# Sliwson/cuda-slam

Measured on AMD Instinct MI355X. Metric: icp_iterations_per_s, higher is better.
Workload: dtype f32

## Files before the change

### cuda-slam_amd/csrc/context.h

```cpp
#pragma once
#include <hip/hip_runtime.h>
#include <rccl/rccl.h>
#include <sys/resource.h>

#include <cstdarg>
#include <cstdio>
#include <string>
#include <vector>

#include "../../include/mi_slam.h"
#include "cpd_kernels.h"
#include "devbuf.h"
#include "kernels.h"
#include "nn_grid.h"
#include "nn_tree.h"

namespace mislam {

void retire_buffers(struct ::mi_ctx* ctx);

#define MI_NCCL(call)                                                                                      \
    do {                                                                                                   \
        ncclResult_t r_ = (call);                                                                          \
        if (r_ != ncclSuccess) {                                                                           \
            mislam::set_error("%s failed: %s (%s:%d)", #call, ncclGetErrorString(r_), __FILE__, __LINE__); \
            return MI_ERR_RCCL;                                                                            \
        }                                                                                                  \
    } while (0)

#define MI_TRY(call)             \
    do {                         \
        int rc_ = (call);        \
        if (rc_ != MI_OK) return rc_; \
    } while (0)

struct GridBuffers {
    DevBuf<float4> pts;
    DevBuf<unsigned int> start, fill, scan;
    DevBuf<unsigned int> slot_of;
    DevBuf<unsigned int> row_occ;
    DevBuf<unsigned char> near_tmp;
};
int grid_reserve(GridBuffers& b, const float bbox[6], int m, int index_base, float points_per_cell, NnGridView* view);
int grid_build_into(GridBuffers& b, const NnGridView& view, const float* x, const float* y, const float* z, int m, hipStream_t s);

struct MortonScratch {
    DevBuf<unsigned int> codes_in, codes_out;
    DevBuf<int> order_in;
    DevBuf<float> bbox;
    DevBuf<unsigned char> sort_temp;
};
int morton_args(MortonScratch& sc, const float* x, const float* y, const float* z, int m, int* order_out, MortonArgs* out);

struct SearchFrontBuffers {
    DevBuf<float> staging;
    DevBuf<float> cx, cy, cz;
    DevBuf<float> ux, uy, uz;
    DevBuf<float> qx, qy, qz;
    DevBuf<float> range_lo_hi;
    DevBuf<int> range_bad;
    DevBuf<KnnState> state;
    DevBuf<int> order;
    MortonScratch morton;
    GridBuffers cells;
    hipEvent_t ev[2] = {nullptr, nullptr};
};

struct ProfileSpan {
    int kernel;
    hipEvent_t e0, e1;
};

struct CpdWorkspace;
struct PrepState;

}

struct mi_ctx {
    int device = 0;
    std::vector<void*> retired;
    unsigned long long entered = 0;
    hipStream_t stream = nullptr;
    int rank = 0, world = 1;
    ncclComm_t comm = nullptr;
    mi_exchange_fn exchange = nullptr;
    void* exchange_user = nullptr;
    void* exchange_host = nullptr;
    size_t exchange_cap = 0;
    bool distributed() const { return comm != nullptr || exchange != nullptr; }
    int cu_count = 256;
    struct Tuning {
        int nn_force_mode = 0;
        int nn_R = 2, nn_wgs = 0, nn_chunks = 0;
        float grid_points_per_cell = mislam::GRID_POINTS_PER_CELL;
        int cpd_mfma = 1;
        int cpd_trunc_cull = 1;
        int fgt_resume = 1;
        int grid_split_walks = -1;
        int grid_deal_rows = -1;
        int svd_ieee = 0;
        int icp_fused_solve = 1;
        int icp_ticket_solve = 1;
        int icp_pipeline = 1;
        int fgt_two_streams = 1;
        int fgt_lists_in_model = 1;
        int fgt_coop_sweep = 1;
        int fgt_shard_queries = 1;
        int fgt_model_splits = 1;
        float knn_points_per_cell = 0.f;
        float outlier_radius_cell = 1.f;
        int fgt_replay = 1;
    } tune;

    hipStream_t aux = nullptr, aux2 = nullptr;
    hipEvent_t aux_event[3] = {nullptr, nullptr, nullptr};
    hipStream_t lane_stream = nullptr;
    int lane = 0;
    hipStream_t work_stream() const { return lane_stream ? lane_stream : stream; }
    struct LaneScratch {
        mislam::DevBuf<float> staging;
        mislam::MortonScratch morton;
    } scratch[2];

    struct PinnedRing {
        static constexpr int SLOTS = 16;
        static constexpr size_t PIECE = 1u << 20;
        char* buf = nullptr;
        hipEvent_t event[SLOTS] = {nullptr};
        unsigned int busy = 0;
        unsigned int next = 0;
    } pin;
    float* h_scratch = nullptr;
    mislam::DevBuf<float> bx, by, bz;
    mislam::DevBuf<float> cx, cy, cz;
    mislam::DevBuf<float> ax, ay, az;
    mislam::DevBuf<float> tx, ty, tz;
    mislam::DevBuf<float4> tgt4;
    mislam::DevBuf<unsigned long long> keys;
    mislam::DevBuf<double> part_mom, part_err;
    struct WorkOrder {
        mislam::DevBuf<int> order, counters;
        mislam::DevBuf<int> ticket;
        mislam::DevBuf<unsigned char> far;
        mislam::DevBuf<unsigned long long> lanes;
    } sched;
    mislam::DevBuf<double> rows, rows_reduced;
    mislam::DevBuf<int> idx_tmp;
    mislam::DevBuf<unsigned char> keep_tmp;
    mislam::IcpState* d_state = nullptr;
    mislam::IcpState* h_state = nullptr;
    hipEvent_t peek_event = nullptr;

    struct TreeIndex {
        mislam::DevBuf<int> order_out;
        mislam::DevBuf<float4> pts, boxes;
        mislam::DevBuf<float4> leaf;
        mislam::DevBuf<int> idx;
        mislam::DevBuf<float> boxes6;
        mislam::NnTreeView view{};
        bool valid = false;
    } tree;
    struct GridIndex {
        mislam::GridBuffers cells;
        mislam::DevBuf<float> bbox;
        mislam::DevBuf<unsigned int> match_slot;
        mislam::NnGridView view{};
        bool valid = false;
    } grid;
    mislam::DevBuf<int> sorder;
    mislam::DevBuf<int> sinv;
    mislam::DevBuf<float> resid;

    struct BatchBuffers {
        mislam::DevBuf<float> before, after, sx, sy, sz;
        mislam::DevBuf<mislam::IcpBatchProblem> problems;
        mislam::DevBuf<mislam::IcpState> states;
        mislam::DevBuf<mislam::CpdBatchProblem> cpd_problems;
        mislam::DevBuf<mislam::CpdState> cpd_states;
        mislam::DevBuf<int> running;
    } bat;

    struct VoxelBuffers {
        mislam::DevBuf<float> staging, x, y, z, range_lo_hi, out_xyz;
        mislam::DevBuf<float4> pts;
        mislam::DevBuf<unsigned int> keys_a, keys_b, axis_keys;
        mislam::DevBuf<int> vals_a, vals_b, range_bad, block_heads, row_of, run_start, fix, out_count, out_coord, voxel_of_point;
        mislam::DevBuf<double> front, back;
        mislam::DevBuf<unsigned char> sort_temp;
        mislam::DevBuf<mislam::VoxState> state;
        double ms[MI_VOXEL_STAGES] = {0};
    } vox;

    struct KnnBuffers {
        mislam::SearchFrontBuffers front;
        mislam::DevBuf<float> out_d2;
        mislam::DevBuf<int> out_idx, out_count;
        double ms[MI_KNN_STAGES] = {0};
    } knn;
    struct NormalsBuffers {
        mislam::SearchFrontBuffers front;
        mislam::DevBuf<float> out_normals, out_curvature;
        mislam::DevBuf<int> out_count;
        double ms[MI_NORMALS_STAGES] = {0};
    } normals;
    struct OutlierBuffers {
        mislam::SearchFrontBuffers front;
        mislam::DevBuf<float> out_xyz, out_mean;
        mislam::DevBuf<int> count, tile_counts, out_index;
        mislam::DevBuf<double> score, partials;
        mislam::DevBuf<unsigned char> keep;
        mislam::DevBuf<mislam::OutlierState> ostate;
        double ms[MI_OUTLIER_STAGES] = {0};
    } outlier;

    struct PrepareBuffers {
        mislam::DevBuf<float> raw, out, partials, noise_unit, outlier_unit;
        mislam::DevBuf<int> sub, shuffle, rows;
        mislam::DevBuf<mislam::PrepState> state;
    } prep;

    struct IcpProblem {
        bool icp_loaded = false;
        int n = 0, n_pad = 0;
        int n_global = 0;
        int m_total = 0, shard_lo = 0, shard_hi = 0;
        bool source_sharded = false;
        bool fused = false;
        int enqueued_passes = 0;
        mi_icp_params icp{};
        double load_ms[MI_LOAD_STAGES] = {0};
    } prob;

    mislam::CpdWorkspace* cpd = nullptr;

    mislam::DevBuf<unsigned long long> nn_stats;
    bool nn_stats_on = false;
    int selftest_fail_loads = 0;
    struct Profiler {
// ... 162 lines not shown
```

### cuda-slam_amd/csrc/mislam_api.hip

```cpp
#include <hip/hip_runtime.h>
#include <dlfcn.h>
#include <rccl/rccl.h>

#include <algorithm>
#include <atomic>
#include <chrono>
#include <cmath>
#include <cstdio>
#include <cstdlib>
#include <cstring>
#include <mutex>
#include <vector>

#include "cloud_range.hpp"
#include "context.h"

using namespace mislam;

namespace mislam {
static thread_local char g_error[512] = "";
void set_error(const char* fmt, ...)
{
    va_list ap;
    va_start(ap, fmt);
// ... 102 lines not shown
        (void)hipMemPoolTrimTo(g_pool[dev], 0);
    }
}
void retire_buffers(mi_ctx* ctx)
{
    std::vector<void*> v;
    v.swap(ctx->retired);
    for (void* p : v) device_free(p);
}
}

double mislam::g_stall_ms = -1.0;

extern "C" const char* mi_last_error(void) { return g_error; }
extern "C" int mi_abi_version(void) { return MI_SLAM_ABI_VERSION; }

extern "C" int mi_device_count(int* count)
{
    if (!count) { set_error("mi_device_count: null argument"); return MI_ERR_INVALID_ARG; }
    int c = 0;
    hipError_t e = hipGetDeviceCount(&c);
    if (e != hipSuccess || c <= 0) {
        *count = 0;
        set_error("no usable HIP device (%s); this library has no CPU fallback", e == hipSuccess ? "count = 0" : hipGetErrorString(e));
        return MI_ERR_NO_DEVICE;
    }
    *count = c;
    return MI_OK;
}

extern "C" int mi_ctx_preload(mi_ctx* c)
{
    if (!c) { set_error("mi_ctx_preload: null context"); return MI_ERR_INVALID_ARG; }
    MI_ENTER(c);
    MI_HIP(preload_nn_kernel()); MI_HIP(preload_nn_tree()); MI_HIP(preload_nn_grid()); MI_HIP(preload_icp_kernels()); MI_HIP(preload_icp_batch()); MI_HIP(preload_cpd_kernels()); MI_HIP(preload_cpd_batch());
    MI_HIP(preload_cpd_fgt()); MI_HIP(preload_nicp_api()); MI_HIP(preload_prepare_api()); MI_HIP(preload_voxel_kernels()); MI_HIP(preload_knn_kernels()); MI_HIP(preload_normals_kernels()); MI_HIP(preload_outlier_kernels());
    return MI_OK;
}

static int ctx_create_common(int device, mi_ctx** out)
{
    if (!out) { set_error("mi_ctx_create: null out pointer"); return MI_ERR_INVALID_ARG; }
    *out = nullptr;
    int count = 0;
    MI_TRY(mi_device_count(&count));
    if (device < 0 || device >= count) { set_error("mi_ctx_create: device %d out of range [0,%d)", device, count); return MI_ERR_INVALID_ARG; }
    MI_HIP(hipSetDevice(device));
    mi_ctx* c = new mi_ctx();
    c->device = device;
    pool_context_created(device);
    const int rc = [&]() -> int {
        hipDeviceProp_t prop;
        MI_HIP(hipGetDeviceProperties(&prop, device));
        c->cu_count = prop.multiProcessorCount > 0 ? prop.multiProcessorCount : 256;
        MI_HIP(hipStreamCreateWithFlags(&c->stream, hipStreamNonBlocking));
        MI_HIP(hipStreamCreateWithFlags(&c->aux, hipStreamNonBlocking));
        MI_HIP(hipStreamCreateWithFlags(&c->aux2, hipStreamNonBlocking));
        for (hipEvent_t& e : c->aux_event) MI_HIP(hipEventCreateWithFlags(&e, hipEventDisableTiming));
        MI_HIP(hipMalloc((void**)&c->d_state, sizeof(IcpState)));
        MI_HIP(hipHostMalloc((void**)&c->h_state, sizeof(IcpState), hipHostMallocDefault));
        MI_HIP(hipEventCreateWithFlags(&c->peek_event, hipEventDisableTiming));
        memset(c->h_state, 0, sizeof(IcpState));
        auto env_i = [](const char* name, int dflt) { const char* v = getenv(name); return (v && *v) ? atoi(v) : dflt; };
        if (const char* sm = getenv("MISLAM_DEV_STALL_MS")) g_stall_ms = atof(sm);
        c->tune.nn_force_mode = env_i("MISLAM_NN_MODE", 0);
        c->tune.nn_R = env_i("MISLAM_NN_R", 2);
        c->tune.nn_wgs = env_i("MISLAM_NN_WGS", 0);
        c->tune.nn_chunks = env_i("MISLAM_NN_CHUNKS", 0);
        c->tune.cpd_mfma = env_i("MISLAM_CPD_MFMA", 1);
        c->tune.cpd_trunc_cull = env_i("MISLAM_CPD_TRUNC_CULL", 1);
        c->tune.fgt_resume = env_i("MISLAM_FGT_RESUME", 1);
        c->tune.fgt_replay = env_i("MISLAM_FGT_REPLAY", 1);
        c->tune.fgt_two_streams = env_i("MISLAM_FGT_TWO_STREAMS", 1);
        c->tune.fgt_lists_in_model = env_i("MISLAM_FGT_LISTS_IN_MODEL", 1);
        c->tune.fgt_coop_sweep = env_i("MISLAM_FGT_COOP_SWEEP", 1);
        c->tune.fgt_model_splits = env_i("MISLAM_FGT_MODEL_SPLITS", 1);
        c->tune.fgt_shard_queries = env_i("MISLAM_FGT_SHARD_QUERIES", 1);
        c->tune.grid_deal_rows = env_i("MISLAM_GRID_DEAL_ROWS", -1);
        c->tune.grid_split_walks = env_i("MISLAM_GRID_SPLIT_WALKS", -1);
        c->tune.icp_pipeline = env_i("MISLAM_ICP_PIPELINE", 1);
        c->tune.icp_fused_solve = env_i("MISLAM_ICP_FUSED_SOLVE", 1);
        c->tune.icp_ticket_solve = env_i("MISLAM_ICP_TICKET_SOLVE", 1);
        c->tune.svd_ieee = env_i("MISLAM_SVD_IEEE", 0);
        if (const char* ppc = getenv("MISLAM_GRID_PPC")) { const float f = (float)atof(ppc); if (f >= 0.25f && f <= 64.f) c->tune.grid_points_per_cell = f; }
        if (const char* ppc = getenv("MISLAM_KNN_POINTS_PER_CELL")) { const float f = (float)atof(ppc); if (f >= 0.125f && f <= 1e30f) c->tune.knn_points_per_cell = f; }
        if (const char* rc = getenv("MISLAM_OUTLIER_RADIUS_CELL")) { const float f = (float)atof(rc); if (f >= 0.125f && f <= 1024.f) c->tune.outlier_radius_cell = f; }
        if (env_i("MISLAM_PRELOAD", 0) == 1) MI_TRY(mi_ctx_preload(c));
        if (env_i("MISLAM_PIN", 0) != 0) {
            MI_HIP(hipHostMalloc((void**)&c->pin.buf, mi_ctx::PinnedRing::PIECE * mi_ctx::PinnedRing::SLOTS, hipHostMallocDefault));
            for (hipEvent_t& e : c->pin.event) MI_HIP(hipEventCreateWithFlags(&e, hipEventDisableTiming));
        }
        MI_HIP(hipHostMalloc((void**)&c->h_scratch, 64 * sizeof(float), hipHostMallocDefault));
        return MI_OK;
    }();
    if (rc != MI_OK) { mi_ctx_destroy(c); return rc; }
    *out = c;
    return MI_OK;
}

extern "C" int mi_ctx_create(int device, mi_ctx** out) { return ctx_create_common(device, out); }

extern "C" int mi_dist_unique_id(void* out_unique_id)
{
    if (!out_unique_id) { set_error("mi_dist_unique_id: null argument"); return MI_ERR_INVALID_ARG; }
    static_assert(sizeof(ncclUniqueId) == MI_UNIQUE_ID_BYTES, "ncclUniqueId size");
    ncclUniqueId id;
    MI_NCCL(ncclGetUniqueId(&id));
    memcpy(out_unique_id, &id, sizeof id);
    return MI_OK;
}

extern "C" int mi_ctx_create_dist(int device, int rank, int world, const void* unique_id, mi_ctx** out)
{
    if (world < 1 || rank < 0 || rank >= world || !unique_id) { set_error("mi_ctx_create_dist: bad rank/world/id"); return MI_ERR_INVALID_ARG; }
    MI_TRY(ctx_create_common(device, out));
    mi_ctx* c = *out;
    c->rank = rank;
    c->world = world;
    ncclUniqueId id;
    memcpy(&id, unique_id, sizeof id);
    ncclResult_t r = ncclCommInitRank(&c->comm, world, id, rank);
    if (r != ncclSuccess) {
        set_error("ncclCommInitRank(rank %d of %d) failed: %s", rank, world, ncclGetErrorString(r));
        mi_ctx_destroy(c);
        *out = nullptr;
        return MI_ERR_RCCL;
    }
    return MI_OK;
}

extern "C" int mi_ctx_create_exchange(int device, int rank, int world, mi_exchange_fn exchange, void* user, mi_ctx** out)
{
    if (world < 1 || rank < 0 || rank >= world || !exchange) { set_error("mi_ctx_create_exchange: bad rank/world/callback"); return MI_ERR_INVALID_ARG; }
    MI_TRY(ctx_create_common(device, out));
    mi_ctx* c = *out;
    c->rank = rank;
    c->world = world;
    c->exchange = exchange;
    c->exchange_user = user;
    return MI_OK;
}

static int exchange_on_host(mi_ctx* c, void* dev_ptr, size_t count, int kind)
{
    const size_t bytes = count * 8;
    if (bytes > c->exchange_cap) {
        if (c->exchange_host) (void)hipHostFree(c->exchange_host);
        c->exchange_host = nullptr;
        c->exchange_cap = 0;
        MI_HIP(hipHostMalloc(&c->exchange_host, bytes, hipHostMallocDefault));
        c->exchange_cap = bytes;
    }
    MI_HIP(hipMemcpyAsync(c->exchange_host, dev_ptr, bytes, hipMemcpyDeviceToHost, c->stream));
    MI_HIP(hipStreamSynchronize(c->stream));
    const int r = c->exchange(c->exchange_user, c->exchange_host, count, kind);
    if (r != 0) { set_error("the exchange callback failed with %d (rank %d of %d, %zu elements, kind %d)", r, c->rank, c->world, count, kind); return MI_ERR_RCCL; }
    MI_HIP(hipMemcpyAsync(dev_ptr, c->exchange_host, bytes, hipMemcpyHostToDevice, c->stream));
    return MI_OK;
}

int mislam::allreduce_min_u64(mi_ctx* c, unsigned long long* dev_ptr, size_t count)
{
    if (c->exchange) return exchange_on_host(c, dev_ptr, count, MI_EXCHANGE_MIN_U64);
    if (!c->comm) return MI_OK;
    MI_NCCL(ncclAllReduce(dev_ptr, dev_ptr, count, ncclUint64, ncclMin, c->comm, c->stream));
    return MI_OK;
// ... 370 lines not shown
```

### cuda-slam_amd/csrc/nn_api.hip

```cpp
#include <hip/hip_runtime.h>

#include <algorithm>
#include <cstring>

#include "context.h"

using namespace mislam;

namespace mislam {

constexpr int NN_MAX_CHUNKS = 1024;

size_t target_alloc_len(int m_local)
{
    return (size_t)round_up(std::max(m_local, 1), NN_TARGET_BLOCK) + (size_t)NN_TARGET_BLOCK * NN_MAX_CHUNKS;
}

NnPlan plan_nn(const mi_ctx* ctx, int n, int m_local)
{
    NnPlan p;
    p.R = ctx->tune.nn_R;
    if (p.R != 1 && p.R != 2 && p.R != 4 && p.R != 8) p.R = 2;
    const int n_src_blocks = round_up(std::max(n, 1), 256 * p.R) / (256 * p.R);
    const int target_wgs = ctx->tune.nn_wgs > 0 ? ctx->tune.nn_wgs : ctx->cu_count * 8;
// ... 29 lines not shown
        c->pin.busy |= 1u << k;
    }
    return MI_OK;
}

int upload_soa(mi_ctx* c, const float* host_aos, int n, int n_pad, float* x, float* y, float* z, float4* packed)
{
    DevBuf<float>& staging = c->scratch[c->lane].staging;
    MI_TRY(staging.reserve((size_t)3 * n));
    MI_TRY(host_to_device(c, staging.p, host_aos, sizeof(float) * 3 * (size_t)n));
    MI_HIP(aos_to_soa(staging.p, n, n_pad, x, y, z, packed, c->work_stream()));
    return MI_OK;
}

int morton_args(MortonScratch& sc, const float* x, const float* y, const float* z, int m, int* order_out, MortonArgs* out)
{
    const size_t sort_bytes = tree_sort_temp_bytes(m);
    MI_TRY(sc.codes_in.reserve((size_t)m)); MI_TRY(sc.codes_out.reserve((size_t)m));
    MI_TRY(sc.order_in.reserve((size_t)m));
    MI_TRY(sc.bbox.reserve(256 * 6 + 8));
    MI_TRY(sc.sort_temp.reserve(sort_bytes + 16));
    MortonArgs a{};
    a.x = x; a.y = y; a.z = z; a.m = m;
    a.bbox_partials = sc.bbox.p; a.bbox = sc.bbox.p + 256 * 6;
    a.codes_in = sc.codes_in.p; a.codes_out = sc.codes_out.p; a.order_in = sc.order_in.p; a.order_out = order_out;
    a.sort_temp = sc.sort_temp.p; a.sort_temp_bytes = sort_bytes;
    *out = a;
    return MI_OK;
}

int grid_reserve(GridBuffers& b, const float bbox[6], int m, int index_base, float points_per_cell, NnGridView* view)
{
    NnGridView g{};
    grid_plan(bbox, m, points_per_cell, &g);
    const size_t n_cells = (size_t)g.nx * g.ny * g.nz;
    MI_TRY(b.pts.reserve((size_t)m + GRID_PTS_PAD));
    MI_TRY(b.row_occ.reserve(n_cells)); MI_TRY(b.near_tmp.reserve(n_cells));
    MI_TRY(b.start.reserve(n_cells + 1 + 3));
    MI_TRY(b.fill.reserve(n_cells + 1));
    MI_TRY(b.scan.reserve((n_cells + 1) / 1024 + 2));
    MI_TRY(b.slot_of.reserve((size_t)m));
    g.pts = b.pts.p;
    g.cell_start = b.start.p;
    g.slot_of = b.slot_of.p;
    g.row_occ = b.row_occ.p;
    g.index_base = index_base;
    *view = g;
    return MI_OK;
}

int grid_build_into(GridBuffers& b, const NnGridView& view, const float* x, const float* y, const float* z, int m, hipStream_t s)
{
    GridBuildArgs a{};
    a.x = x; a.y = y; a.z = z; a.m = m; a.index_base = view.index_base;
    a.view = view; a.cell_fill = b.fill.p; a.scan_tmp = b.scan.p; a.pts_out = b.pts.p; a.cell_start_out = b.start.p; a.slot_of_out = b.slot_of.p;
    a.row_occ_out = b.row_occ.p; a.near_tmp = b.near_tmp.p;
    MI_HIP(grid_build(a, s));
    return MI_OK;
}

int ensure_tree(mi_ctx* c, int m_local, int index_base)
{
    if (c->tree.valid) return MI_OK;
    const int n_leaves = (m_local + TREE_LEAF - 1) / TREE_LEAF;
    int n_pad = 1, height = 0;
    while (n_pad < n_leaves) { n_pad <<= 1; height++; }
    if (height > TREE_MAX_HEIGHT) { set_error("fixed cloud too large for the box hierarchy"); return MI_ERR_INVALID_ARG; }
    if (c->selftest_fail_loads > 0) {
        c->selftest_fail_loads -= 1;
        set_error("index build failed on request (mi_selftest_fail_loads)");
        return MI_ERR_INVALID_ARG;
    }
    MI_TRY(c->tree.order_out.reserve((size_t)m_local));
    MI_TRY(c->tree.pts.reserve((size_t)n_leaves * TREE_LEAF));
    MI_TRY(c->tree.boxes.reserve((size_t)4 * n_pad));
    MI_TRY(c->tree.leaf.reserve((size_t)n_leaves * (3 * TREE_LEAF / 4)));
    MI_TRY(c->tree.idx.reserve((size_t)n_leaves * TREE_LEAF));
    MI_TRY(c->tree.boxes6.reserve((size_t)12 * ((size_t)n_pad + 6)));
    TreeBuildArgs a{};
    MI_TRY(morton_args(c->scratch[c->lane].morton, c->tx.p, c->ty.p, c->tz.p, m_local, c->tree.order_out.p, &a.morton));
    a.index_base = index_base; a.n_leaves = n_leaves; a.n_pad = n_pad;
    a.pts = c->tree.pts.p; a.boxes = c->tree.boxes.p;
    a.leaf_soa = c->tree.leaf.p; a.leaf_idx = c->tree.idx.p; a.boxes6 = c->tree.boxes6.p;
    MI_HIP(tree_build(a, c->work_stream()));
    c->tree.view.boxes6 = c->tree.boxes6.p;
    c->tree.view.leaf_soa = c->tree.leaf.p; c->tree.view.leaf_idx = c->tree.idx.p;
    c->tree.view.n_pad = n_pad; c->tree.view.height = height; c->tree.view.n_leaves = n_leaves;
    c->tree.valid = true;
    return MI_OK;
}

int ensure_grid(mi_ctx* c, int m_local, int index_base)
{
    if (c->grid.valid) return MI_OK;
    const hipStream_t ws = c->work_stream();
    MI_TRY(c->grid.bbox.reserve(256 * 6 + 8));
    float* d_bbox = c->grid.bbox.p + 256 * 6;
    MI_HIP(cloud_bbox(c->tx.p, c->ty.p, c->tz.p, m_local, c->grid.bbox.p, d_bbox, ws));
    float* bbox = c->h_scratch;
    MI_HIP(hipMemcpyAsync(bbox, d_bbox, 6 * sizeof(float), hipMemcpyDeviceToHost, ws));
    { StallProbe sp("grid: bounding-box synchronize"); MI_HIP(hipStreamSynchronize(ws)); }
    StallProbe sp_rest("grid: reserve + enqueue build");
    NnGridView g{};
    MI_TRY(grid_reserve(c->grid.cells, bbox, m_local, index_base, c->tune.grid_points_per_cell, &g));
    MI_TRY(grid_build_into(c->grid.cells, g, c->tx.p, c->ty.p, c->tz.p, m_local, ws));
    c->grid.view = g;
    c->grid.valid = true;
    return MI_OK;
}

int reserve_moving(mi_ctx* c, size_t n_pad, size_t c_pad)
{
    MI_TRY(c->bx.reserve(n_pad)); MI_TRY(c->by.reserve(n_pad)); MI_TRY(c->bz.reserve(n_pad));
    MI_TRY(c->cx.reserve(c_pad)); MI_TRY(c->cy.reserve(c_pad)); MI_TRY(c->cz.reserve(c_pad));
    return c->keys.reserve(n_pad);
}

int sort_sources(mi_ctx* c, const float* sx, const float* sy, const float* sz, int n, int n_pad, float* dx, float* dy, float* dz)
{
    MI_TRY(c->sorder.reserve((size_t)n));
    MortonArgs ma{};
    MI_TRY(morton_args(c->scratch[c->lane].morton, sx, sy, sz, n, c->sorder.p, &ma));
    MI_HIP(morton_order(ma, c->work_stream()));
    MI_HIP(permute_soa(sx, sy, sz, c->sorder.p, n, n_pad, dx, dy, dz, c->work_stream()));
    return MI_OK;
}

int resolve_nn_mode(const mi_ctx* c, int nn_mode, int m_local)
{
    const int forced = c->tune.nn_force_mode;
    if (forced == MI_NN_BRUTEFORCE || forced == MI_NN_TREE || forced == MI_NN_GRID) nn_mode = forced;
    if (nn_mode == MI_NN_BRUTEFORCE || nn_mode == MI_NN_TREE || nn_mode == MI_NN_GRID) return nn_mode;
    return m_local >= MI_NN_INDEX_MIN_POINTS ? MI_NN_GRID : MI_NN_BRUTEFORCE;
}

extern "C" const char* mi_nn_kernel_name(const mi_ctx* c, int n_moving, int m_fixed_local, int nn_mode)
{
    (void)n_moving;
    if (!c) return "";
    const int mode = resolve_nn_mode(c, nn_mode, m_fixed_local);
    return mode == MI_NN_GRID ? nn_grid_kernel_name(false) : (mode == MI_NN_TREE ? "nn_tree_kernel" : "nn_bruteforce_kernel");
}

GridSearchArgs grid_search_args(const mi_ctx* c, int n)
{
    GridSearchArgs a{};
    a.n = n; a.keys = c->keys.p;
    a.stats = c->nn_stats_on ? c->nn_stats.p : nullptr;
    a.deal_rows = c->tune.grid_deal_rows < 0 ? (n >= GRID_DEAL_ROWS_MIN_POINTS ? 1 : 0) : c->tune.grid_deal_rows;
    return a;
}

int launch_nn(mi_ctx* c, const float* sx, const float* sy, const float* sz, int n, int m_local, int index_base, int fma,
                      const int* done_flag, int nn_mode)
{
    const int mode = resolve_nn_mode(c, nn_mode, m_local);
    if (mode == MI_NN_TREE || mode == MI_NN_GRID) {
        MI_TRY(ensure_tree(c, m_local, index_base));
        if (mode == MI_NN_GRID) MI_TRY(ensure_grid(c, m_local, index_base));
        ProfScope ps(c, MI_KERNEL_NN);
        if (mode == MI_NN_GRID) {
            GridSearchArgs a = grid_search_args(c, n);
            a.sx = sx; a.sy = sy; a.sz = sz; a.done_flag = done_flag;
            MI_HIP(nn_grid_query(c->grid.view, c->tree.view, a, fma, c->stream));
        } else {
            MI_HIP(nn_tree_query(c->tree.view, sx, sy, sz, n, c->keys.p, done_flag, fma, c->stream));
        }
// ... 80 lines not shown
```

### cuda-slam_amd/csrc/nn_tree.hip

```cpp
#include <hip/hip_runtime.h>

#include "cloud_range.hpp"
#include "kernels.h"
#include "nn_tree.h"
#include "nn_walk.hpp"
#include "curve_code.hpp"

namespace mislam {
__global__ __launch_bounds__(256) void tree_bbox_partial_kernel(const float* __restrict__ x, const float* __restrict__ y,
                                                                const float* __restrict__ z, int m, float* __restrict__ partials)
{
    range_block(SoaPoints{x, y, z}, AnyPoint{}, m, partials, nullptr);
}

__global__ __launch_bounds__(256) void tree_bbox_final_kernel(const float* __restrict__ partials, int nblocks, float* __restrict__ bbox)
{
    RangeAcc a;
    if (!range_finish<0>(a, partials, nblocks)) return;
#pragma unroll
    for (int k = 0; k < 6; k++) bbox[k] = a.v[k];
}

__global__ __launch_bounds__(256) void tree_morton_kernel(const float* __restrict__ x, const float* __restrict__ y,
                                                          const float* __restrict__ z, int m, const float* __restrict__ bbox,
                                                          unsigned int* __restrict__ codes, int* __restrict__ order)
{
    const int j = blockIdx.x * 256 + threadIdx.x;
    if (j >= m) return;
    const float p[3] = {x[j], y[j], z[j]};
    codes[j] = curve_code30(p, bbox);
    order[j] = j;
}

size_t tree_sort_temp_bytes(int m) { return radix_sort_temp_bytes(m); }

hipError_t cloud_bbox(const float* x, const float* y, const float* z, int m, float* partials, float* bbox, hipStream_t s)
{
    const int rb = range_blocks(m, 256);
    hipLaunchKernelGGL(tree_bbox_partial_kernel, dim3(rb), dim3(256), 0, s, x, y, z, m, partials);
    hipLaunchKernelGGL(tree_bbox_final_kernel, dim3(1), dim3(256), 0, s, partials, rb, bbox);
    return hipGetLastError();
}

hipError_t morton_order(const MortonArgs& a, hipStream_t s)
{
    const int m = a.m;
    const int blocks = (m + 255) / 256;
    hipError_t be = cloud_bbox(a.x, a.y, a.z, m, a.bbox_partials, a.bbox, s);
    if (be != hipSuccess) return be;
    hipLaunchKernelGGL(tree_morton_kernel, dim3(blocks), dim3(256), 0, s, a.x, a.y, a.z, m, a.bbox, a.codes_in, a.order_in);
    return radix_sort_pairs_u32(a.sort_temp, a.codes_in, a.codes_out, a.order_in, a.order_out, m, 30, s);
}

__global__ __launch_bounds__(256) void permute_soa_kernel(const float* __restrict__ x, const float* __restrict__ y,
                                                          const float* __restrict__ z, const int* __restrict__ order, int m, int n_out,
                                                          float* __restrict__ ox, float* __restrict__ oy, float* __restrict__ oz)
{
    const int s = blockIdx.x * 256 + threadIdx.x;
    if (s >= n_out) return;
    const int j = order[s < m ? s : m - 1];
    ox[s] = x[j]; oy[s] = y[j]; oz[s] = z[j];
}

hipError_t permute_soa(const float* x, const float* y, const float* z, const int* order, int m, int n_out, float* ox, float* oy,
                       float* oz, hipStream_t s)
{
    if (n_out <= 0) return hipSuccess;
    hipLaunchKernelGGL(permute_soa_kernel, dim3((n_out + 255) / 256), dim3(256), 0, s, x, y, z, order, m, n_out, ox, oy, oz);
    return hipGetLastError();
}

__global__ __launch_bounds__(256) void tree_gather_kernel(const float* __restrict__ x, const float* __restrict__ y,
                                                          const float* __restrict__ z, const int* __restrict__ order, int m,
                                                          int n_slots, int index_base, float4* __restrict__ pts)
{
    const int s = blockIdx.x * 256 + threadIdx.x;
    if (s >= n_slots) return;
    const int j = order[s < m ? s : m - 1];
    pts[s] = make_float4(x[j], y[j], z[j], __int_as_float(j + index_base));
}

__global__ __launch_bounds__(256) void tree_leaf_box_kernel(const float4* __restrict__ pts, int n_leaves, int n_pad, float4* __restrict__ boxes)
{
    const int leaf = blockIdx.x * 256 + threadIdx.x;
    if (leaf >= n_pad) return;
    float lo[3] = {__builtin_inff(), __builtin_inff(), __builtin_inff()};
    float hi[3] = {-__builtin_inff(), -__builtin_inff(), -__builtin_inff()};
    if (leaf < n_leaves) {
        for (int k = 0; k < TREE_LEAF; k++) {
            const float4 p = pts[(size_t)leaf * TREE_LEAF + k];
            lo[0] = fminf(lo[0], p.x); lo[1] = fminf(lo[1], p.y); lo[2] = fminf(lo[2], p.z);
            hi[0] = fmaxf(hi[0], p.x); hi[1] = fmaxf(hi[1], p.y); hi[2] = fmaxf(hi[2], p.z);
        }
    }
    const size_t node = (size_t)(n_pad - 1 + leaf);
    boxes[2 * node] = make_float4(lo[0], lo[1], lo[2], 0.f);
    boxes[2 * node + 1] = make_float4(hi[0], hi[1], hi[2], 0.f);
}

__global__ __launch_bounds__(256) void tree_level_kernel(int first, int count, float4* __restrict__ boxes)
{
    const int i = blockIdx.x * 256 + threadIdx.x;
    if (i >= count) return;
    const size_t node = (size_t)(first + i), l = 2 * node + 1, r = l + 1;
    const float4 a = boxes[2 * l], c = boxes[2 * l + 1], b = boxes[2 * r], d = boxes[2 * r + 1];
    boxes[2 * node] = make_float4(fminf(a.x, b.x), fminf(a.y, b.y), fminf(a.z, b.z), 0.f);
    boxes[2 * node + 1] = make_float4(fmaxf(c.x, d.x), fmaxf(c.y, d.y), fmaxf(c.z, d.z), 0.f);
}

__global__ __launch_bounds__(256) void tree_pack_boxes6_kernel(const float4* __restrict__ boxes, int n_nodes, int n_out, float* __restrict__ boxes6)
{
    const int i = blockIdx.x * 256 + threadIdx.x;
    if (i >= n_out) return;
    float4 lo = make_float4(__builtin_inff(), __builtin_inff(), __builtin_inff(), 0.f);
    float4 hi = make_float4(-__builtin_inff(), -__builtin_inff(), -__builtin_inff(), 0.f);
    if (i == 0) {
        float* e = boxes6;
        e[0] = lo.x; e[2] = lo.y; e[4] = lo.z; e[6] = hi.x; e[8] = hi.y; e[10] = hi.z;
    }
    if (i < n_nodes) { lo = boxes[2 * (size_t)i]; hi = boxes[2 * (size_t)i + 1]; }
    float* o = boxes6 + tree_box_offset(i);
    o[0] = lo.x; o[2] = lo.y; o[4] = lo.z; o[6] = hi.x; o[8] = hi.y; o[10] = hi.z;
}

__global__ __launch_bounds__(256) void tree_pack_leaves_kernel(const float4* __restrict__ pts, int n_slots, float* __restrict__ soa,
                                                               int* __restrict__ idx)
{
    const int s = blockIdx.x * 256 + threadIdx.x;
    if (s >= n_slots) return;
    const float4 q = pts[s];
    const int leaf = s / TREE_LEAF, k = s % TREE_LEAF;
    float* base = soa + (size_t)leaf * 3 * TREE_LEAF;
    base[k] = q.x; base[TREE_LEAF + k] = q.y; base[2 * TREE_LEAF + k] = q.z;
    idx[s] = __float_as_int(q.w);
}

hipError_t tree_build(const TreeBuildArgs& a, hipStream_t s)
{
    hipError_t e = morton_order(a.morton, s);
    if (e != hipSuccess) return e;
    const int m = a.morton.m;
    const int n_slots = a.n_leaves * TREE_LEAF;
    hipLaunchKernelGGL(tree_gather_kernel, dim3((n_slots + 255) / 256), dim3(256), 0, s, a.morton.x, a.morton.y, a.morton.z,
                       a.morton.order_out, m, n_slots, a.index_base, a.pts);
    hipLaunchKernelGGL(tree_leaf_box_kernel, dim3((a.n_pad + 255) / 256), dim3(256), 0, s, a.pts, a.n_leaves, a.n_pad, a.boxes);
    for (int count = a.n_pad / 2; count >= 1; count /= 2)
        hipLaunchKernelGGL(tree_level_kernel, dim3((count + 255) / 256), dim3(256), 0, s, count - 1, count, a.boxes);
    const int n_nodes = 2 * a.n_pad - 1;
    hipLaunchKernelGGL(tree_pack_boxes6_kernel, dim3((n_nodes + 8 + 255) / 256), dim3(256), 0, s, a.boxes, n_nodes, n_nodes + 8, a.boxes6);
    hipLaunchKernelGGL(tree_pack_leaves_kernel, dim3((n_slots + 255) / 256), dim3(256), 0, s, a.pts, n_slots, reinterpret_cast<float*>(a.leaf_soa),
                       a.leaf_idx);
    return hipGetLastError();
}

template <bool FMA>
__global__ __launch_bounds__(TREE_BLOCK_THREADS) void nn_tree_kernel(NnTreeView t, const float* __restrict__ sx, const float* __restrict__ sy,
                                                                          const float* __restrict__ sz, int n, unsigned long long* __restrict__ keys,
                                                                          const int* __restrict__ done_flag)
{
    if (done_flag != nullptr && *done_flag != 0) return;
    const unsigned int chunk = xcd_chunk(blockIdx.x, gridDim.x, TREE_XCD_CHUNKS * (256 / TREE_BLOCK_THREADS));
    const int i = (int)(chunk * TREE_BLOCK_THREADS + threadIdx.x);
    if (i >= n) return;
    const float p[3] = {sx[i], sy[i], sz[i]};
    float best;
    unsigned int bidx;
    unpack_start(keys[i], best, bidx);
    unsigned int n_nodes = 0u, n_leaves = 0u;
    tree_walk_wide<FMA, false>(t, p, best, bidx, n_nodes, n_leaves);
    if (best < __builtin_inff()) keys[i] = ((unsigned long long)__float_as_uint(best) << 32) | bidx;
}

hipError_t nn_tree_query(const NnTreeView& t, const float* sx, const float* sy, const float* sz, int n, unsigned long long* keys,
                         const int* done_flag, int fma, hipStream_t s)
{
    if (n <= 0) return hipSuccess;
    const dim3 grid((n + TREE_BLOCK_THREADS - 1) / TREE_BLOCK_THREADS), block(TREE_BLOCK_THREADS);
    if (fma) hipLaunchKernelGGL(nn_tree_kernel<true>, grid, block, 0, s, t, sx, sy, sz, n, keys, done_flag);
    else hipLaunchKernelGGL(nn_tree_kernel<false>, grid, block, 0, s, t, sx, sy, sz, n, keys, done_flag);
    return hipGetLastError();
}

__global__ void preload_nn_tree_kernel() {}
hipError_t preload_nn_tree()
{
    hipFuncAttributes attr;
    return hipFuncGetAttributes(&attr, reinterpret_cast<const void*>(preload_nn_tree_kernel));
}

}
```

Before: 26060.

## Build NN tree with median-split kd ordering instead of Morton curve order

Adds a kd-style point ordering for the NN tree build. Upper levels split segments along their widest axis using per-segment bounding boxes and radix sorts, and lower levels use an in-LDS bitonic sort per 2048-slot block. The build then reuses the existing gather/box code. It is enabled by default, with the old Hilbert/Morton path selectable by env var. The goal is tighter leaf boxes and so cheaper NN traversal, at the cost of a heavier tree build with many more kernel launches.

```diff
diff --git a/cuda-slam_amd/csrc/context.h b/cuda-slam_amd/csrc/context.h
--- a/cuda-slam_amd/csrc/context.h
+++ b/cuda-slam_amd/csrc/context.h
@@ -14,6 +14,7 @@
 #include "kernels.h"
 #include "nn_grid.h"
 #include "nn_tree.h"
+#include "tree_order.h"
 
 namespace mislam {
 
@@ -109,6 +110,7 @@
         int fgt_model_splits = 1;
         float knn_points_per_cell = 0.f;
         float outlier_radius_cell = 1.f;
+        int tree_order = mislam::TREE_ORDER_KD;
         int fgt_replay = 1;
     } tune;
 
@@ -154,6 +156,7 @@
     struct TreeIndex {
         mislam::DevBuf<int> order_out;
         mislam::DevBuf<float4> pts, boxes;
+        mislam::DevBuf<unsigned int> seg_box;
         mislam::DevBuf<float4> leaf;
         mislam::DevBuf<int> idx;
         mislam::DevBuf<float> boxes6;
diff --git a/cuda-slam_amd/csrc/mislam_api.hip b/cuda-slam_amd/csrc/mislam_api.hip
--- a/cuda-slam_amd/csrc/mislam_api.hip
+++ b/cuda-slam_amd/csrc/mislam_api.hip
@@ -208,6 +208,11 @@
         c->tune.icp_fused_solve = env_i("MISLAM_ICP_FUSED_SOLVE", 1);
         c->tune.icp_ticket_solve = env_i("MISLAM_ICP_TICKET_SOLVE", 1);
         c->tune.svd_ieee = env_i("MISLAM_SVD_IEEE", 0);
+        if (const char* to = getenv("MISLAM_TREE_ORDER")) {
+            if (strcmp(to, "hilbert") == 0) c->tune.tree_order = TREE_ORDER_HILBERT;
+            else if (strcmp(to, "kd") == 0 || *to == 0) c->tune.tree_order = TREE_ORDER_KD;
+            else { set_error("MISLAM_TREE_ORDER: hilbert or kd"); return MI_ERR_INVALID_ARG; }
+        }
         if (const char* ppc = getenv("MISLAM_GRID_PPC")) { const float f = (float)atof(ppc); if (f >= 0.25f && f <= 64.f) c->tune.grid_points_per_cell = f; }
         if (const char* ppc = getenv("MISLAM_KNN_POINTS_PER_CELL")) { const float f = (float)atof(ppc); if (f >= 0.125f && f <= 1e30f) c->tune.knn_points_per_cell = f; }
         if (const char* rc = getenv("MISLAM_OUTLIER_RADIUS_CELL")) { const float f = (float)atof(rc); if (f >= 0.125f && f <= 1024.f) c->tune.outlier_radius_cell = f; }
diff --git a/cuda-slam_amd/csrc/nn_api.hip b/cuda-slam_amd/csrc/nn_api.hip
--- a/cuda-slam_amd/csrc/nn_api.hip
+++ b/cuda-slam_amd/csrc/nn_api.hip
@@ -135,7 +135,14 @@
     a.index_base = index_base; a.n_leaves = n_leaves; a.n_pad = n_pad;
     a.pts = c->tree.pts.p; a.boxes = c->tree.boxes.p;
     a.leaf_soa = c->tree.leaf.p; a.leaf_idx = c->tree.idx.p; a.boxes6 = c->tree.boxes6.p;
-    MI_HIP(tree_build(a, c->work_stream()));
+    if (c->tune.tree_order == TREE_ORDER_KD) {
+        TreeOrderArgs o{};
+        MI_TRY(c->tree.seg_box.reserve(kd_seg_box_words(n_pad)));
+        o.seg_box = c->tree.seg_box.p;
+        MI_HIP(tree_build_kd(a, o, c->work_stream()));
+    } else {
+        MI_HIP(tree_build(a, c->work_stream()));
+    }
     c->tree.view.boxes6 = c->tree.boxes6.p;
     c->tree.view.leaf_soa = c->tree.leaf.p; c->tree.view.leaf_idx = c->tree.idx.p;
     c->tree.view.n_pad = n_pad; c->tree.view.height = height; c->tree.view.n_leaves = n_leaves;
diff --git a/cuda-slam_amd/csrc/nn_tree.hip b/cuda-slam_amd/csrc/nn_tree.hip
--- a/cuda-slam_amd/csrc/nn_tree.hip
+++ b/cuda-slam_amd/csrc/nn_tree.hip
@@ -5,6 +5,7 @@
 #include "nn_tree.h"
 #include "nn_walk.hpp"
 #include "curve_code.hpp"
+#include "tree_order.h"
 
 namespace mislam {
 __global__ __launch_bounds__(256) void tree_bbox_partial_kernel(const float* __restrict__ x, const float* __restrict__ y,
@@ -139,6 +140,11 @@
 {
     hipError_t e = morton_order(a.morton, s);
     if (e != hipSuccess) return e;
+    return tree_build_from_order(a, s);
+}
+
+hipError_t tree_build_from_order(const TreeBuildArgs& a, hipStream_t s)
+{
     const int m = a.morton.m;
     const int n_slots = a.n_leaves * TREE_LEAF;
     hipLaunchKernelGGL(tree_gather_kernel, dim3((n_slots + 255) / 256), dim3(256), 0, s, a.morton.x, a.morton.y, a.morton.z,
diff --git a/cuda-slam_amd/csrc/tree_order.h b/cuda-slam_amd/csrc/tree_order.h
--- /dev/null
+++ b/cuda-slam_amd/csrc/tree_order.h
@@ -0,0 +1,26 @@
+#pragma once
+#include <hip/hip_runtime.h>
+
+#include "nn_tree.h"
+
+namespace mislam {
+
+constexpr int TREE_ORDER_HILBERT = 0, TREE_ORDER_KD = 1;
+constexpr int KD_BLOCK_SLOTS = 2048;
+
+__host__ inline int kd_upper_levels(int n_pad)
+{
+    int levels = 0;
+    for (long long cap = (long long)n_pad * TREE_LEAF; cap > KD_BLOCK_SLOTS; cap >>= 1) levels++;
+    return levels;
+}
+__host__ inline size_t kd_seg_box_words(int n_pad) { return 6 * ((size_t)1 << kd_upper_levels(n_pad)); }
+
+struct TreeOrderArgs {
+    unsigned int* seg_box;
+};
+
+hipError_t tree_build_from_order(const TreeBuildArgs& a, hipStream_t s);
+hipError_t tree_build_kd(const TreeBuildArgs& a, const TreeOrderArgs& o, hipStream_t s);
+
+}
diff --git a/cuda-slam_amd/csrc/tree_order.hip b/cuda-slam_amd/csrc/tree_order.hip
--- /dev/null
+++ b/cuda-slam_amd/csrc/tree_order.hip
@@ -0,0 +1,194 @@
+#include <hip/hip_runtime.h>
+
+#include "kernels.h"
+#include "nn_tree.h"
+#include "tree_order.h"
+
+namespace mislam {
+
+__device__ __forceinline__ unsigned int kd_ordered(float f)
+{
+    const unsigned int b = __float_as_uint(f);
+    return (b & 0x80000000u) ? ~b : (b | 0x80000000u);
+}
+__device__ __forceinline__ float kd_unordered(unsigned int u)
+{
+    return __uint_as_float((u & 0x80000000u) ? (u & 0x7fffffffu) : ~u);
+}
+
+__device__ __forceinline__ unsigned int kd_coordinate(const float (&p)[3], const float (&lo)[3], const float (&hi)[3])
+{
+    int axis = 0;
+    float ext = hi[0] - lo[0];
+    if (hi[1] - lo[1] > ext) { axis = 1; ext = hi[1] - lo[1]; }
+    if (hi[2] - lo[2] > ext) { axis = 2; ext = hi[2] - lo[2]; }
+    const float pa = axis == 0 ? p[0] : (axis == 1 ? p[1] : p[2]);
+    const float la = axis == 0 ? lo[0] : (axis == 1 ? lo[1] : lo[2]);
+    float u = ext > 0.f ? (pa - la) / ext : 0.f;
+    u = fminf(fmaxf(u * 1024.f, 0.f), 1023.f);
+    return (unsigned int)u;
+}
+
+__global__ __launch_bounds__(256) void kd_seg_box_init_kernel(unsigned int* __restrict__ seg_box, int n_segs)
+{
+    const int i = blockIdx.x * 256 + threadIdx.x;
+    if (i >= n_segs * 6) return;
+    seg_box[i] = (i % 6) < 3 ? 0xffffffffu : 0u;
+}
+
+__global__ __launch_bounds__(256) void kd_seg_box_kernel(const float* __restrict__ x, const float* __restrict__ y, const float* __restrict__ z,
+                                                         const int* __restrict__ order, int m, int cap_shift, unsigned int* __restrict__ seg_box)
+{
+    __shared__ unsigned int red[6];
+    const int first = blockIdx.x * 1024;
+    if (threadIdx.x < 6) red[threadIdx.x] = threadIdx.x < 3 ? 0xffffffffu : 0u;
+    __syncthreads();
+    unsigned int lo[3] = {0xffffffffu, 0xffffffffu, 0xffffffffu}, hi[3] = {0u, 0u, 0u};
+    for (int k = 0; k < 4; k++) {
+        const int i = first + k * 256 + (int)threadIdx.x;
+        if (i < m) {
+            const int j = order ? order[i] : i;
+            const unsigned int c[3] = {kd_ordered(x[j]), kd_ordered(y[j]), kd_ordered(z[j])};
+#pragma unroll
+            for (int a = 0; a < 3; a++) { lo[a] = c[a] < lo[a] ? c[a] : lo[a]; hi[a] = c[a] > hi[a] ? c[a] : hi[a]; }
+        }
+    }
+#pragma unroll
+    for (int o = 32; o >= 1; o >>= 1)
+#pragma unroll
+        for (int a = 0; a < 3; a++) {
+            const unsigned int l2 = (unsigned int)__shfl_xor((int)lo[a], o, 64), h2 = (unsigned int)__shfl_xor((int)hi[a], o, 64);
+            lo[a] = l2 < lo[a] ? l2 : lo[a]; hi[a] = h2 > hi[a] ? h2 : hi[a];
+        }
+    if ((threadIdx.x & 63) == 0)
+#pragma unroll
+        for (int a = 0; a < 3; a++) { atomicMin(&red[a], lo[a]); atomicMax(&red[3 + a], hi[a]); }
+    __syncthreads();
+    if (threadIdx.x < 6 && first < m) {
+        unsigned int* b = seg_box + (size_t)(first >> cap_shift) * 6;
+        if (threadIdx.x < 3) atomicMin(&b[threadIdx.x], red[threadIdx.x]);
+        else atomicMax(&b[threadIdx.x], red[threadIdx.x]);
+    }
+}
+
+__global__ __launch_bounds__(256) void kd_key_kernel(const float* __restrict__ x, const float* __restrict__ y, const float* __restrict__ z,
+                                                     const int* __restrict__ order, int m, int cap_shift, const unsigned int* __restrict__ seg_box,
+                                                     unsigned int* __restrict__ keys, int* __restrict__ vals)
+{
+    const int i = blockIdx.x * 256 + threadIdx.x;
+    if (i >= m) return;
+    const int j = order ? order[i] : i;
+    const unsigned int seg = (unsigned int)i >> cap_shift;
+    const unsigned int* b = seg_box + (size_t)seg * 6;
+    const float lo[3] = {kd_unordered(b[0]), kd_unordered(b[1]), kd_unordered(b[2])};
+    const float hi[3] = {kd_unordered(b[3]), kd_unordered(b[4]), kd_unordered(b[5])};
+    const float p[3] = {x[j], y[j], z[j]};
+    keys[i] = (seg << 10) | kd_coordinate(p, lo, hi);
+    vals[i] = j;
+}
+
+constexpr int KD_T = 256;
+constexpr int KD_OWN = KD_BLOCK_SLOTS / KD_T;
+static_assert(KD_OWN == 8 && TREE_LEAF % KD_OWN == 0, "a thread's positions lie in one leaf, so in one node of every level");
+__global__ __launch_bounds__(KD_T) void kd_block_kernel(const float* __restrict__ x, const float* __restrict__ y, const float* __restrict__ z,
+                                                        const int* __restrict__ order_in, int m, int block_slots, int* __restrict__ order_out)
+{
+    __shared__ float px[KD_BLOCK_SLOTS], py[KD_BLOCK_SLOTS], pz[KD_BLOCK_SLOTS];
+    __shared__ int pj[KD_BLOCK_SLOTS];
+    __shared__ unsigned int key[KD_BLOCK_SLOTS];
+    __shared__ unsigned short perm_a[KD_BLOCK_SLOTS], perm_b[KD_BLOCK_SLOTS];
+    __shared__ unsigned int box[(KD_BLOCK_SLOTS / 16) * 6];
+    const int t = threadIdx.x;
+    const int first = blockIdx.x * block_slots;
+    const int cnt = m - first < block_slots ? m - first : block_slots;
+    for (int i = t; i < KD_BLOCK_SLOTS; i += KD_T) {
+        if (i < cnt) {
+            const int j = order_in ? order_in[first + i] : first + i;
+            px[i] = x[j]; py[i] = y[j]; pz[i] = z[j]; pj[i] = j;
+        }
+        perm_a[i] = (unsigned short)i;
+    }
+    __syncthreads();
+    unsigned short* perm = perm_a;
+    unsigned short* perm_next = perm_b;
+    for (int cap = block_slots; cap >= 16; cap >>= 1) {
+        const int n_nodes = block_slots / cap;
+        for (int i = t; i < n_nodes * 6; i += KD_T) box[i] = (i % 6) < 3 ? 0xffffffffu : 0u;
+        __syncthreads();
+        const int own = t * KD_OWN;
+        if (own < cnt) {
+            unsigned int lo[3] = {0xffffffffu, 0xffffffffu, 0xffffffffu}, hi[3] = {0u, 0u, 0u};
+            for (int k = 0; k < KD_OWN && own + k < cnt; k++) {
+                const int q = perm[own + k];
+                const unsigned int c[3] = {kd_ordered(px[q]), kd_ordered(py[q]), kd_ordered(pz[q])};
+#pragma unroll
+                for (int a = 0; a < 3; a++) { lo[a] = c[a] < lo[a] ? c[a] : lo[a]; hi[a] = c[a] > hi[a] ? c[a] : hi[a]; }
+            }
+            unsigned int* b = box + (own / cap) * 6;
+#pragma unroll
+            for (int a = 0; a < 3; a++) { atomicMin(&b[a], lo[a]); atomicMax(&b[3 + a], hi[a]); }
+        }
+        __syncthreads();
+        for (int k = 0; k < KD_OWN; k++) {
+            const int i = own + k;
+            unsigned int coord = 1024u;
+            if (i < cnt) {
+                const unsigned int* b = box + (i / cap) * 6;
+                const float lo[3] = {kd_unordered(b[0]), kd_unordered(b[1]), kd_unordered(b[2])};
+                const float hi[3] = {kd_unordered(b[3]), kd_unordered(b[4]), kd_unordered(b[5])};
+                const int q = perm[i];
+                const float p[3] = {px[q], py[q], pz[q]};
+                coord = kd_coordinate(p, lo, hi);
+            }
+            key[i] = (coord << 11) | (unsigned int)i;
+        }
+        __syncthreads();
+        for (int k = 2; k <= cap; k <<= 1)
+            for (int j = k >> 1; j > 0; j >>= 1) {
+                for (int e = t; e < block_slots / 2; e += KD_T) {
+                    const int i = ((e & ~(j - 1)) << 1) | (e & (j - 1)), l = i | j;
+                    const bool up = k == cap || (i & k) == 0;
+                    const unsigned int a = key[i], b = key[l];
+                    if ((a > b) == up) { key[i] = b; key[l] = a; }
+                }
+                __syncthreads();
+            }
+        for (int i = t; i < block_slots; i += KD_T) perm_next[i] = perm[key[i] & (KD_BLOCK_SLOTS - 1)];
+        __syncthreads();
+        unsigned short* sw = perm; perm = perm_next; perm_next = sw;
+    }
+    for (int i = t; i < cnt; i += KD_T) order_out[first + i] = pj[perm[i]];
+}
+
+hipError_t tree_build_kd(const TreeBuildArgs& a, const TreeOrderArgs& o, hipStream_t s)
+{
+    const MortonArgs& ma = a.morton;
+    const int m = ma.m;
+    if (m <= 0) return hipErrorInvalidValue;
+    const long long n_slots_pad = (long long)a.n_pad * TREE_LEAF;
+    const int upper = kd_upper_levels(a.n_pad);
+    if (upper > 20 || m > n_slots_pad) return hipErrorInvalidValue;
+    const int* cur = nullptr;
+    if (upper > 0) {
+        const int n_segs = 1 << upper;
+        hipLaunchKernelGGL(kd_seg_box_init_kernel, dim3((n_segs * 6 + 255) / 256), dim3(256), 0, s, o.seg_box, n_segs);
+        int cap_shift = 0;
+        while ((1ll << cap_shift) < n_slots_pad) cap_shift++;
+        for (int level = 0; level < upper; level++, cap_shift--) {
+            unsigned int* boxes = o.seg_box + (size_t)((1 << level) - 1) * 6;
+            hipLaunchKernelGGL(kd_seg_box_kernel, dim3((m + 1023) / 1024), dim3(256), 0, s, ma.x, ma.y, ma.z, cur, m, cap_shift, boxes);
+            hipLaunchKernelGGL(kd_key_kernel, dim3((m + 255) / 256), dim3(256), 0, s, ma.x, ma.y, ma.z, cur, m, cap_shift, boxes, ma.codes_in,
+                               ma.order_in);
+            hipError_t e = radix_sort_pairs_u32(ma.sort_temp, ma.codes_in, ma.codes_out, ma.order_in, ma.order_out, m, level + 10, s);
+            if (e != hipSuccess) return e;
+            cur = ma.order_out;
+        }
+    }
+    const int block_slots = n_slots_pad < KD_BLOCK_SLOTS ? (int)n_slots_pad : KD_BLOCK_SLOTS;
+    hipLaunchKernelGGL(kd_block_kernel, dim3((m + block_slots - 1) / block_slots), dim3(KD_T), 0, s, ma.x, ma.y, ma.z, cur, m, block_slots, ma.order_out);
+    hipError_t e = hipGetLastError();
+    if (e != hipSuccess) return e;
+    return tree_build_from_order(a, s);
+}
+
+}
```

After: 26010. About the same (-0.2%).
